# simonrw/rust-tensorflow-serving2

Measured on AMD Instinct MI355X. Metric: Predict RPCs/sec + p50 latency, ResNet-50 batch=1/32 at 1/2/4/8 MI355X, higher is better.
Workload: dtype bf16

## Files before the change

rust_tensorflow_serving2_amd/graph/fused.py:

```python
from __future__ import annotations

import os
from typing import Dict, List, Optional, Sequence, Set, Tuple

import numpy as np
import torch
import torch.nn.functional as F

from ..utils import tensors as T
from . import ops as O
from .ir import Graph, Node
from .placement import to_device, zeros

BF16 = torch.bfloat16


def _const(g: Graph, ref) -> Optional[torch.Tensor]:
    n = g.nodes.get(ref[0])
    if n is None or n.op != "Const" or n.value is None:
        return None
    v = n.value[ref[1]] if ref[1] < len(n.value) else None
    return v if isinstance(v, torch.Tensor) else None


# ... 686 lines not shown
        hc = (x.shape[1] + pt + pb - conv.kh) // conv.sh + 1
        wc = (x.shape[2] + pl + pr - conv.kw) // conv.sw + 1
        if pool.padding == "SAME":
            (ppt, ppb), (ppl, ppr) = O.tf_same_pads(hc, 3, 2), O.tf_same_pads(wc, 3, 2)
        else:
            ppt = ppb = ppl = ppr = 0
        kw = {}
        if pool.post is not None:
            sc, sh, act = pool.post
            kw = dict(post_scale=sc, post_shift=sh, post_act=ACT[act])
        x = x.contiguous() if x.dtype == torch.bfloat16 else x.float().contiguous()
        return [hip().stem_pool(x, conv.w, conv.b, pt, pb, pl, pr, ACT[conv.act],
                                ppt, ppb, ppl, ppr, **kw)]


O.OPS["_StemPool"] = _impl_op

CHAIN_SHAPES_ALL = {(64, 256, 64), (64, 256, 128), (128, 512, 128), (128, 512, 256)}
CHAIN_SHAPES_STAGE1 = {(64, 256, 64), (64, 256, 128)}
CHAIN_SHAPES_DEFAULT = CHAIN_SHAPES_ALL


class ChainConv:

    children = ("a", "b")

    def __init__(self, a: FusedConv, b: FusedConv):
        self.a, self.b = a, b
        self.use_hip = a.use_hip and b.use_hip
        self.name = a.name

    def __call__(self, ctx, node, ins):
        x = O.to_torch(ins[0])
        res = O.to_torch(ins[1]) if len(ins) > 1 else None
        a, b = self.a, self.b

        def split():
            y1 = a(ctx, node, ins)[0]
            return [y1, b(ctx, node, [y1])[0]]
        if not (self.use_hip and x.is_cuda and x.dim() == 4 and x.shape[-1] == a.cin):
            return split()
        from ..ops import ACT, hip, tuned_choice
        xb = _to_bf16(x).contiguous()
        rb = None if res is None else _to_bf16(res).contiguous()

        def chained():
            return list(hip().conv_chain(xb, a.w, a.b, rb, ACT[a.act], b.w, b.b, ACT[b.act]))
        key = ("chain", tuple(x.shape), a.cout, b.cout, res is not None, a.act, b.act)
        dflt = 1 if (a.cin, a.cout, b.cout) in CHAIN_SHAPES_STAGE1 else 0
        pick = tuned_choice(key, {1: chained, 0: split}, default=dflt)
        return chained() if pick == 1 else split()


O.OPS["_ChainConv"] = _impl_op
O.OPS["_FusedMatMulLN"] = _impl_op

_PASSTHROUGH = ("Identity", "Squeeze", "Reshape")


def fuse_classifier_head(g, order, fed, fetch_refs, device, opts):
    c = _Ctx(g, order, fed, fetch_refs, device, opts)

    def single(node) -> bool:
        return node.name not in c.fetch_nodes and len(c.cons.get(node.name, [])) == 1

    def walk(ref, chain):
        n = g.nodes.get(ref[0])
        while n is not None and n.op in _PASSTHROUGH and ref[1] == 0 and single(n) and n.inputs:
            chain.append(n)
            ref = n.inputs[0]
            n = g.nodes.get(ref[0])
        return ref, n

    for name in order:
        sm = g.nodes.get(name)
        if sm is None or sm.op != "_SoftmaxArgMax" or not sm.inputs:
            continue
        chain: List[Node] = []
        ref, mm = walk(sm.inputs[0], chain)
        if mm is None or mm.op != "_FusedMatMul" or ref[1] != 0 or len(mm.inputs) != 1 or not single(mm):
            continue
        impl = mm.attrs["_impl"]
        if impl.act != "none":
            continue
        chain.append(mm)
        ref, gap = walk(mm.inputs[0], chain)
        if gap is None or gap.op != "_GlobalAvgPool" or ref[1] != 0 or not single(gap):
            continue
        chain.append(gap)
        sm_impl = sm.attrs["_impl"]
        head = ClassifierHead(impl, sm_impl.cdt, c.use_hip)
        sm.op = "_ClassifierHead"
        sm.inputs = [gap.inputs[0]]
        sm.attrs = {"_impl": head}
        sm.ctrl = _merge_ctrl(chain + [sm])
        for n in chain:
            del g.nodes[n.name]
        c.refresh()


def fuse_stem_pool(g, order, fed, fetch_refs, device, opts):
    import os
    if os.environ.get("TFSERVE_STEM_POOL", "1") == "0":
        return
    c = _Ctx(g, order, fed, fetch_refs, device, opts)
    for name in order:
        p = g.nodes.get(name)
# ... 279 lines not shown
        impl = p.attrs["_impl"]
        if impl.post is not None or not impl.post_ok() or name in c.fetch_nodes:
            continue
        cons = c.cons.get(name, [])
        if any(i != 0 for _c, _p, i in cons):
            continue
        bns = [g.nodes[cn] for cn, _pos, _i in cons
               if g.nodes[cn].op.startswith("FusedBatchNorm") and g.nodes[cn].inputs[0] == (name, 0)]
        if len(bns) != 1:
            continue
        bn = bns[0]
        aff = _bn_affine(g, c, bn)
        if aff is None or aff[0].numel() != getattr(impl, "cout", aff[0].numel()):
            continue
        out_node, act = bn, "none"
        relu = c.only_consumer(bn.name)
        if relu is not None and relu.op == "Relu" and relu.name not in c.fetch_nodes:
            out_node, act = relu, "relu"
        elif bn.name in c.fetch_nodes:
            continue
        others = [cn for cn, _pos, _i in cons if cn != bn.name]
        if isinstance(impl, MaxPool) and others:
            continue
        mode = "dual" if others else "only"
        if isinstance(impl, MaxPool):
            impl.set_post(aff[0], aff[1], act, mode, device=c.device)
        else:
            impl.set_post(aff[0], aff[1], act, mode)
        new_ref = (name, 1 if mode == "dual" else 0)
        for cn, pos, _i in c.cons.get(out_node.name, []):
            g.nodes[cn].inputs[pos] = new_ref
        p.ctrl = _merge_ctrl([p, bn] + ([out_node] if out_node is not bn else []))
        del g.nodes[bn.name]
        if out_node is not bn:
            del g.nodes[out_node.name]
        c.refresh()


def _chainable_1x1(impl) -> bool:
    return (isinstance(impl, FusedConv) and impl.kh == 1 and impl.kw == 1 and impl.sh == 1 and impl.sw == 1 and
            not impl.c4 and impl.post is None and impl.act in ("relu", "none") and
            (impl.padding != "EXPLICIT" or not any(impl.pads)))


def fuse_conv_chain(g, order, fed, fetch_refs, device, opts):
    import os
    mode = os.environ.get("TFSERVE_CONV_CHAIN", "1")
    shapes = CHAIN_SHAPES_STAGE1 if os.environ.get("TFSERVE_CONV_CHAIN_SHAPES") == "stage1" else CHAIN_SHAPES_ALL
    c = _Ctx(g, order, fed, fetch_refs, device, opts)
    if mode == "0" or (not c.use_hip and mode != "force"):
        return
    for name in order:
        p = g.nodes.get(name)
        if p is None or p.op != "_FusedConv2D" or name in c.fetch_nodes:
            continue
        a = p.attrs["_impl"]
        if not _chainable_1x1(a):
            continue
        cons = c.cons.get(name, [])
        if any(i != 0 for _c, _p, i in cons):
            continue
        bs = [g.nodes[cn] for cn, pos, _i in cons
              if pos == 0 and g.nodes[cn].op == "_FusedConv2D" and len(g.nodes[cn].inputs) == 1 and
              cn not in c.fetch_nodes and _chainable_1x1(g.nodes[cn].attrs["_impl"])]
        if len(bs) != 1:
            continue
        bnode = bs[0]
        b = bnode.attrs["_impl"]
        if b.cin != a.cout or (a.cin, a.cout, b.cout) not in shapes:
            continue
        chain = ChainConv(a, b)
        p.op = "_ChainConv"
        p.attrs = {"_impl": chain}
        for cn, pos, _i in c.cons.get(bnode.name, []):
            g.nodes[cn].inputs[pos] = (name, 1)
        p.ctrl = _merge_ctrl([p, bnode])
        del g.nodes[bnode.name]
        c.refresh()


def default_passes(options=None):
    from .patterns import bert_passes, late_passes
    return [fuse_pools, fuse_softmax_argmax] + bert_passes() + [fuse_conv, fuse_dual_conv, fuse_post_activation,
                                                                 fuse_stem_pool, fuse_matmul,
                                                                 fuse_classifier_head, fuse_dense_softmax,
                                                                 fuse_conv_chain] + late_passes() + \
        [fuse_matmul_layernorm, defer_layernorm, release_weight_sources]
```

rust_tensorflow_serving2_amd/kernels/bindings.cpp:

```cpp
#include <cstdlib>
#include <algorithm>
#include <torch/extension.h>
#include <ATen/hip/impl/HIPGuardImplMasqueradingAsCUDA.h>
#include <ATen/hip/impl/HIPStreamMasqueradingAsCUDA.h>

#include "launch.h"
#include "cgemm.h"

namespace {

using torch::Tensor;

hipStream_t cur_stream(const Tensor& t) {
  return c10::hip::getCurrentHIPStreamMasqueradingAsCUDA(t.device().index()).stream();
}

void check(hipError_t e, const char* what) {
  TORCH_CHECK(e == hipSuccess, what, ": ", hipGetErrorString(e));
}

bool is_cgemm_cfg(int64_t cfg) {
  return cfg >= 0 && cfg < (1 << 20) && tfsk::cgemm_cfg_id(int(cfg));
}

// ... 375 lines not shown
    sh = post_shift->data_ptr<float>();
  }
  check(tfsk::maxpool_nhwc_launch(bf16p(x), bf16p_mut(y), N, H, W, C, KH, KW, SH, SW, PT, PL, Ho, Wo,
                                  cur_stream(x), sc, sh, int(post_act)), "maxpool");
  return y;
}

Tensor stem_pool(const Tensor& x, const Tensor& w, const Tensor& bias, int64_t PT, int64_t PB, int64_t PL, int64_t PR,
                 int64_t act, int64_t PPT, int64_t PPB, int64_t PPL, int64_t PPR,
                 const c10::optional<Tensor>& post_scale, const c10::optional<Tensor>& post_shift, int64_t post_act) {
  const bool xb16 = x.scalar_type() == at::kBFloat16;
  need(x, xb16 ? at::kBFloat16 : at::kFloat, "x");
  need(w, at::kBFloat16, "w");
  need(bias, at::kFloat, "bias");
  TORCH_CHECK(x.dim() == 4 && x.size(3) >= 1 && x.size(3) <= 4, "stem_pool: x must be NHWC with C <= 4");
  TORCH_CHECK(w.dim() == 2 && w.size(0) % 16 == 0 && w.size(0) >= 16 && w.size(0) <= 64 && w.size(1) >= 224 &&
              w.size(1) % 8 == 0, "stem_pool: w must be [cout in 16..64 step 16][>= 224, % 8]");
  TORCH_CHECK(bias.numel() == w.size(0), "stem_pool: bias must have cout entries");
  TORCH_CHECK(PT >= 0 && PB >= 0 && PL >= 0 && PR >= 0 && PPT >= 0 && PPT <= 2 && PPL >= 0 && PPL <= 2 &&
              PPB >= 0 && PPR >= 0, "stem_pool: bad padding");
  TORCH_CHECK(w.device() == x.device() && bias.device() == x.device(), "stem_pool: tensors on different devices");
  Tensor xin = x;
  if (xb16 && x.numel() % 2) {
    const int64_t avail = int64_t(x.storage().nbytes()) - int64_t(x.storage_offset()) * 2;
    if (avail < x.numel() * 2 + 2 || !x.is_contiguous()) {
      Tensor padded = torch::zeros({x.numel() + 1}, x.options());
      padded.narrow(0, 0, x.numel()).copy_(x.reshape({-1}));
      xin = padded.narrow(0, 0, x.numel()).view(x.sizes());
    }
  }
  c10::hip::HIPGuardMasqueradingAsCUDA guard(x.device());
  const int N = x.size(0), H = x.size(1), W = x.size(2), C = x.size(3), cout = w.size(0);
  const int Hc = (H + PT + PB - 7) / 2 + 1, Wc = (W + PL + PR - 7) / 2 + 1;
  TORCH_CHECK(Hc >= 1 && Wc >= 1, "stem_pool: input smaller than the filter");
  const int Hp = (Hc + PPT + PPB - 3) / 2 + 1, Wp = (Wc + PPL + PPR - 3) / 2 + 1;
  TORCH_CHECK(Hp >= 1 && Wp >= 1, "stem_pool: conv output smaller than the pool window");
  Tensor y = torch::empty({N, Hp, Wp, cout}, x.options().dtype(at::kBFloat16));
  const float* sc = nullptr;
  const float* sh = nullptr;
  if (post_scale.has_value()) {
    TORCH_CHECK(post_shift.has_value(), "post_scale needs post_shift");
    need(*post_scale, at::kFloat, "post_scale");
    need(*post_shift, at::kFloat, "post_shift");
    TORCH_CHECK(post_scale->numel() == cout && post_shift->numel() == cout, "post scale / shift must have cout entries");
    sc = post_scale->data_ptr<float>();
    sh = post_shift->data_ptr<float>();
  }
  check(tfsk::stem_pool_launch(xin.data_ptr(), xb16, bf16p(w), int(w.size(1)), bias.data_ptr<float>(), bf16p_mut(y), N,
                               H, W, C, cout, int(PT), int(PL), Hc, Wc, int(PPT), int(PPL), Hp, Wp, int(act), sc, sh,
                               int(post_act), cur_stream(x)), "stem_pool");
  return y;
}

std::vector<Tensor> conv_chain(const Tensor& x, const Tensor& w1, const Tensor& b1,
                               const c10::optional<Tensor>& residual, int64_t act1, const Tensor& w2,
                               const Tensor& b2, int64_t act2) {
  need(x, at::kBFloat16, "x");
  need(w1, at::kBFloat16, "w1");
  need(w2, at::kBFloat16, "w2");
  need(b1, at::kFloat, "b1");
  need(b2, at::kFloat, "b2");
  TORCH_CHECK(x.dim() == 4, "conv_chain: x must be NHWC");
  const int K1 = x.size(3), N1 = w1.size(0), N2 = w2.size(0);
  TORCH_CHECK(w1.dim() == 2 && w2.dim() == 2 && w1.size(1) >= K1 && w2.size(1) >= N1 && w1.size(1) % 8 == 0 &&
                  w2.size(1) % 8 == 0, "conv_chain: w1 [N1][>= K1], w2 [N2][>= N1]");
  TORCH_CHECK(tfsk::conv_chain_supported(K1, N1, N2), "conv_chain: unsupported shape K1=", K1, " N1=", N1, " N2=", N2);
  TORCH_CHECK(b1.numel() == N1 && b2.numel() == N2, "conv_chain: bias sizes");
  TORCH_CHECK(w1.device() == x.device() && w2.device() == x.device() && b1.device() == x.device() &&
                  b2.device() == x.device(), "conv_chain: tensors on different devices");
  const uint16_t* rp = nullptr;
  if (residual.has_value()) {
    need(*residual, at::kBFloat16, "residual");
    TORCH_CHECK(residual->dim() == 4 && residual->size(0) == x.size(0) && residual->size(1) == x.size(1) &&
                    residual->size(2) == x.size(2) && residual->size(3) == N1, "conv_chain: residual [n][h][w][N1]");
    rp = bf16p(*residual);
  }
  c10::hip::HIPGuardMasqueradingAsCUDA guard(x.device());
  const int M = x.size(0) * x.size(1) * x.size(2);
  Tensor y1 = torch::empty({x.size(0), x.size(1), x.size(2), N1}, x.options());
  Tensor y2 = torch::empty({x.size(0), x.size(1), x.size(2), N2}, x.options());
  check(tfsk::conv_chain_launch(bf16p(x), bf16p(w1), int(w1.size(1)), b1.data_ptr<float>(), rp, bf16p_mut(y1),
                                bf16p(w2), int(w2.size(1)), b2.data_ptr<float>(), bf16p_mut(y2), M, K1, N1, N2,
                                int(act1), int(act2), cur_stream(x)),
        "conv_chain");
  return {y1, y2};
}

Tensor global_avgpool(const Tensor& x, const c10::optional<Tensor>& out) {
  need(x, at::kBFloat16, "x");
  TORCH_CHECK(x.dim() == 4 && x.size(3) % 8 == 0, "global_avgpool: NHWC with C % 8 == 0");
  c10::hip::HIPGuardMasqueradingAsCUDA guard(x.device());
  const int N = x.size(0), HW = x.size(1) * x.size(2), C = x.size(3);
  Tensor y = out.has_value() ? *out : torch::empty({N, C}, x.options());
  need(y, at::kBFloat16, "out");
  check(tfsk::global_avgpool_nhwc_launch(bf16p(x), bf16p_mut(y), N, HW, C, cur_stream(x)), "gap");
  return y;
}

std::vector<Tensor> softmax_argmax(const Tensor& logits, bool want_probs, bool want_classes,
                                   const c10::optional<Tensor>& probs_out,
                                   const c10::optional<Tensor>& classes_out) {
  TORCH_CHECK(logits.is_cuda() && logits.dim() >= 1 && logits.stride(-1) == 1 &&
                  (logits.is_contiguous() || logits.dim() == 2),
              "logits must be a GPU tensor with unit column stride (contiguous, or 2-D with a row stride)");
  const bool bf = logits.scalar_type() == at::kBFloat16;
  TORCH_CHECK(bf || logits.scalar_type() == at::kFloat, "logits must be f32 or bf16");
  c10::hip::HIPGuardMasqueradingAsCUDA guard(logits.device());
  const int cols = logits.size(-1);
  const int rows = logits.numel() / cols;
  const long ld = logits.dim() == 2 ? long(logits.stride(0)) : long(cols);
  TORCH_CHECK(ld >= cols, "logits row stride");
  Tensor probs, classes;
  if (want_probs) {
    probs = probs_out.has_value() ? *probs_out : torch::empty(logits.sizes(), logits.options().dtype(at::kFloat));
    need(probs, at::kFloat, "probs");
  }
  if (want_classes) {
    auto sz = logits.sizes().vec();
    sz.pop_back();
    classes = classes_out.has_value() ? *classes_out : torch::empty(sz, logits.options().dtype(at::kLong));
    need(classes, at::kLong, "classes");
  }
  check(tfsk::softmax_argmax_launch(logits.data_ptr(), bf, want_probs ? probs.data_ptr<float>() : nullptr,
                                    want_classes ? classes.data_ptr<int64_t>() : nullptr, rows, cols, ld,
                                    cur_stream(logits)), "softmax_argmax");
  return {probs, classes};
}

std::tuple<Tensor, Tensor, bool> classifier_head_impl(const Tensor& x, const Tensor& w, const Tensor& bias, int64_t n,
                                                      int64_t probs_host, int64_t classes_host);

std::vector<Tensor> classifier_head(const Tensor& x, const Tensor& w, const Tensor& bias, int64_t n) {
  auto r = classifier_head_impl(x, w, bias, n, 0, 0);
  return {std::get<0>(r), std::get<1>(r)};
}

std::tuple<Tensor, Tensor, bool> classifier_head_impl(const Tensor& x, const Tensor& w, const Tensor& bias, int64_t n,
// ... 182 lines not shown
  }
  if (pos.has_value()) {
    need(*pos, at::kBFloat16, "pos");
    TORCH_CHECK(pos->dim() == 2 && pos->size(1) == Hd && pos->size(0) >= seq, "embed_ln: pos shape");
    pp = bf16p(*pos);
  }
  auto shape = ids.sizes().vec();
  shape.push_back(Hd);
  Tensor y = torch::empty(shape, word.options());
  check(tfsk::embed_ln_launch(ids.data_ptr<int>(), tt, bf16p(word), pp, tp, gamma.data_ptr<float>(),
                              beta.data_ptr<float>(), bf16p_mut(y), tokens, seq, Hd, word.size(0), ntypes,
                              float(eps), cur_stream(ids)), "embed_ln");
  return y;
}

Tensor attention(const Tensor& qkv, const c10::optional<Tensor>& mask_bias, int64_t heads, double scale,
                 const c10::optional<Tensor>& out, int64_t mask_bstride, int64_t mask_qstride) {
  need(qkv, at::kBFloat16, "qkv");
  TORCH_CHECK(qkv.dim() == 3, "qkv must be [B, S, 3*H*D]");
  c10::hip::HIPGuardMasqueradingAsCUDA guard(qkv.device());
  const int B = qkv.size(0), S = qkv.size(1), HD3 = qkv.size(2);
  TORCH_CHECK(HD3 % (3 * heads) == 0, "qkv width must be 3*heads*head_dim");
  const int D = HD3 / (3 * heads);
  TORCH_CHECK(D == 64, "attention kernel supports head_dim 64");
  TORCH_CHECK(S >= 1 && S <= tfsk::kMaxAttentionSeq, "attention kernel supports 1 <= S <= ", tfsk::kMaxAttentionSeq);
  const float* mb = nullptr;
  if (mask_bias.has_value()) {
    need(*mask_bias, at::kFloat, "mask_bias");
    const int64_t last = int64_t(B - 1) * mask_bstride + int64_t(S - 1) * mask_qstride + (S - 1);
    TORCH_CHECK(mask_bstride >= 0 && mask_qstride >= 0 && last < mask_bias->numel(),
                "mask strides exceed the mask tensor");
    mb = mask_bias->data_ptr<float>();
  }
  Tensor y = out.has_value() ? *out : torch::empty({B, S, heads * D}, qkv.options());
  need(y, at::kBFloat16, "out");
  check(tfsk::attention_launch(bf16p(qkv), mb, bf16p_mut(y), B, S, heads, D, float(scale), mask_bstride,
                               mask_qstride, cur_stream(qkv)),
        "attention");
  return y;
}

}

PYBIND11_MODULE(TORCH_EXTENSION_NAME, m) {
  m.doc() = "gfx950 HIP kernels (MFMA implicit-GEMM conv/GEMM, attention, norms, pooling)";
  m.def("conv2d", &conv2d, "NHWC implicit-GEMM conv (+bias +residual +act)", py::arg("x"), py::arg("w"),
        py::arg("bias"), py::arg("residual"), py::arg("kh"), py::arg("kw"), py::arg("sh"), py::arg("sw"),
        py::arg("pt"), py::arg("pb"), py::arg("pl"), py::arg("pr"), py::arg("act") = 0, py::arg("cfg") = 0,
        py::arg("out") = py::none(), py::arg("out_f32") = false, py::arg("splits") = 1,
        py::arg("post_scale") = py::none(), py::arg("post_shift") = py::none(), py::arg("post_act") = 0,
        py::arg("out2") = py::none(), py::arg("post_only") = false);
  m.def("conv_chain", &conv_chain, "expand 1x1 (+residual, act) -> next reduce 1x1 (+act) in one kernel",
        py::arg("x"), py::arg("w1"), py::arg("b1"), py::arg("residual"), py::arg("act1"), py::arg("w2"),
        py::arg("b2"), py::arg("act2"));
  m.def("conv_chain_supported", [](int64_t k1, int64_t n1, int64_t n2) {
    return tfsk::conv_chain_supported(int(k1), int(n1), int(n2));
  });
  m.def("conv2d_dual", &conv2d_dual, "act(conv1x1(h) + conv1x1_stride(x) + bias) as one K-concatenated GEMM",
        py::arg("h"), py::arg("x"), py::arg("w"), py::arg("bias"), py::arg("sh"), py::arg("sw"), py::arg("act") = 0,
        py::arg("cfg") = 36, py::arg("out") = py::none(), py::arg("splits") = 1,
        py::arg("post_scale") = py::none(), py::arg("post_shift") = py::none(), py::arg("post_act") = 0,
        py::arg("out2") = py::none(), py::arg("post_only") = false);
  m.def("linear_lnx", &linear_lnx,
        "GEMM whose A / residual rows are LayerNorm inputs (statistics as partials), optionally "
        "returning its own rows' partials: {y, partials}",
        py::arg("x"), py::arg("w"), py::arg("bias"), py::arg("residual"), py::arg("act"), py::arg("cfg"),
        py::arg("out_f32") = false, py::arg("out") = py::none(), py::arg("a_st") = py::none(),
        py::arg("a_colsum") = py::none(), py::arg("a_eps") = 1e-12, py::arg("r_st") = py::none(),
        py::arg("r_gamma") = py::none(), py::arg("r_beta") = py::none(), py::arg("r_eps") = 1e-12,
        py::arg("stats") = false);
  m.def("linear", &linear,"x @ w^T (+bias +residual +act)", py::arg("x"), py::arg("w"), py::arg("bias"),
        py::arg("residual") = py::none(), py::arg("act") = 0, py::arg("cfg") = 0, py::arg("out_f32") = false,
        py::arg("alpha") = 1.0, py::arg("out") = py::none(), py::arg("splits") = 1);
  m.def("stem_pool", &stem_pool, py::arg("x"), py::arg("w"), py::arg("bias"), py::arg("pt"), py::arg("pb"),
        py::arg("pl"), py::arg("pr"), py::arg("act"), py::arg("ppt"), py::arg("ppb"), py::arg("ppl"), py::arg("ppr"),
        py::arg("post_scale") = py::none(), py::arg("post_shift") = py::none(), py::arg("post_act") = 0);
  m.def("maxpool", &maxpool, py::arg("x"), py::arg("kh"), py::arg("kw"), py::arg("sh"), py::arg("sw"),
        py::arg("pt"), py::arg("pb"), py::arg("pl"), py::arg("pr"), py::arg("out") = py::none(),
        py::arg("post_scale") = py::none(), py::arg("post_shift") = py::none(), py::arg("post_act") = 0);
  m.def("global_avgpool", &global_avgpool, py::arg("x"), py::arg("out") = py::none());
  m.def("classifier_head", &classifier_head, "softmax/argmax(mean_hw(x) @ w^T + bias)[:, :n]", py::arg("x"),
        py::arg("w"), py::arg("bias"), py::arg("n"));
  m.def("softmax_argmax", &softmax_argmax, py::arg("logits"), py::arg("want_probs") = true,
        py::arg("want_classes") = true, py::arg("probs_out") = py::none(), py::arg("classes_out") = py::none());
  m.def("dense_softmax", &dense_softmax, "softmax(x @ w[:n]^T + bias[:n]) for n <= 16 labels (x f32)",
        py::arg("x"), py::arg("w"), py::arg("bias"), py::arg("n"));
  m.def("key_mask_adder", &key_mask_adder, "(one - m) * scale as f32", py::arg("m"), py::arg("one"),
        py::arg("scale"));
  m.def("cast_bf16", &cast_bf16, py::arg("x"), py::arg("out") = py::none());
  m.def("ingest_c4", &ingest_c4, "fp32 NHWC (C<=4) -> bf16 NHWC C=4", py::arg("x"), py::arg("out") = py::none());
  m.def("ingest_c4_padded", &ingest_c4_padded, "fp32 NHWC (C<=4) -> zero-bordered bf16 RGBA [N][Hp][Wp][4]",
        py::arg("x"), py::arg("hp"), py::arg("wp"), py::arg("pt"), py::arg("pl"));
  m.def("ingest_c4_from_host", &ingest_c4_from_host, "ingest_c4 reading a pinned host tensor (zero-copy)",
        py::arg("x"), py::arg("out"));
  m.def("h2d_rows", &h2d_rows, py::arg("host"), py::arg("dev"),
        "copy a pinned host tensor into a device tensor with a kernel (system-scope loads; capturable)");
  m.def("cast_bf16_from_host", &cast_bf16_from_host, "fp32 pinned host tensor -> bf16 device tensor",
        py::arg("x"), py::arg("out"));
  m.def("linear_ln", &linear_ln, "LN(x @ w^T + bias + residual) * gamma + beta, whole rows per workgroup",
        py::arg("x"), py::arg("w"), py::arg("bias"), py::arg("residual"), py::arg("gamma"), py::arg("beta"),
        py::arg("eps"), py::arg("bm") = 32, py::arg("out") = py::none());
  m.def("linear_ln_supported", [](int64_t M, int64_t N, int64_t K, int64_t bm) {
    return tfsk::lngemm_supported(int(M), int(N), int(K), int(bm));
  });
  m.def("layernorm", &layernorm, py::arg("x"), py::arg("residual"), py::arg("gamma"), py::arg("beta"),
        py::arg("eps"), py::arg("out") = py::none());
  m.def("embed_ln", &embed_ln, py::arg("ids"), py::arg("type_ids"), py::arg("word"), py::arg("pos"),
// ... 70 lines not shown
```

rust_tensorflow_serving2_amd/kernels/chain.hip:

```cpp
#include "gemm_common.h"

namespace tfsk {
namespace {

using namespace gemm;

struct ChainArgs {
  const uint16_t* x;
  const uint16_t* w1;
  const float* b1;
  const uint16_t* res;
  uint16_t* y1;
  const uint16_t* w2;
  const float* b2;
  uint16_t* y2;
  int M, ldw1, ldw2;
  float lo1, lo2;
};

constexpr int kBM = 64, kNT = 256, kStgLd = 68;

template <int K1, int N1, int N2>
struct CH {
  static constexpr int KT1 = K1 / KT, KT2 = N1 / KT;
  static constexpr int A_BYTES = KT1 * kBM * KT * 2;
  static constexpr int W1_BYTES = KT1 * N1 * KT * 2;
  static constexpr int P1 = A_BYTES + W1_BYTES;
  static constexpr int CHAIN = KT2 * kBM * KT * 2;
  static constexpr int STG = 4 * 16 * kStgLd * 4;
  static constexpr int S2 = N2 <= 128 ? 3 : 2;
  static constexpr int W2_SLOT = N2 * KT * 2;
  static constexpr int RING_OFF = CHAIN;
  static constexpr int P23 = CHAIN + (STG > S2 * W2_SLOT ? STG : S2 * W2_SLOT);
  static constexpr int LDS = P1 > P23 ? P1 : P23;
  static constexpr int WN1 = N1 / 4, TN1 = WN1 / 16, U1 = WN1 / 64;
  static constexpr int WN2 = N2 / 2, TN2 = WN2 / 16;
  static constexpr int UW2 = WN2 < 64 ? WN2 : 64, U2 = WN2 / UW2;
  static constexpr int APW = KT1 * (kBM / 8) / 4, W1PW = KT1 * (N1 / 8) / 4, W2PW = N2 / 32;
  static_assert(K1 % KT == 0 && N1 % 256 == 0 && N2 % 64 == 0, "chain shape");
  static_assert(LDS <= 160 * 1024, "LDS budget");
  static_assert((S2 - 2) * W2PW < 64, "vmcnt range");
};

template <int K1, int N1, int N2>
__global__ __launch_bounds__(256, 1) void conv_chain_kernel(ChainArgs p) {
  using G = CH<K1, N1, N2>;
  extern __shared__ __attribute__((aligned(16))) char smem[];
  typedef __attribute__((address_space(3))) void* lds_ptr_t;
  const int tid = threadIdx.x, lane = tid & 63;
  const int wid = __builtin_amdgcn_readfirstlane(tid >> 6);
  const int fr = lane & 15, fq = lane >> 4;
  const int prow = lane >> 3;
  const uint32_t kc = uint32_t(((lane & 7) ^ prow) * 8);
  const int m0 = xcd_remap(blockIdx.x, gridDim.x) * kBM;
  const int M = p.M;

  const __amdgpu_buffer_rsrc_t rsX = __builtin_amdgcn_make_buffer_rsrc(
      const_cast<uint16_t*>(p.x), 0, int(long(M) * K1 * 2), 0x00020000);
  const __amdgpu_buffer_rsrc_t rsW1 = __builtin_amdgcn_make_buffer_rsrc(
      const_cast<uint16_t*>(p.w1), 0, int(long(N1) * p.ldw1 * 2), 0x00020000);
  const __amdgpu_buffer_rsrc_t rsW2 = __builtin_amdgcn_make_buffer_rsrc(
      const_cast<uint16_t*>(p.w2), 0, int(long(N2) * p.ldw2 * 2), 0x00020000);

#pragma unroll
  for (int j = 0; j < G::APW; ++j) {
    const int q = wid * G::APW + j;
    const int kt = q / (kBM / 8), pc = q % (kBM / 8);
    const int m = m0 + pc * 8 + prow;
    const uint32_t v = m < M ? (uint32_t(m) * K1 + uint32_t(kt * KT) + kc) * 2u : kOOB;
    __builtin_amdgcn_raw_ptr_buffer_load_lds(rsX, (lds_ptr_t)(smem + kt * kBM * KT * 2 + pc * 1024), 16, v, 0, 0, 0);
  }
#pragma unroll
  for (int j = 0; j < G::W1PW; ++j) {
    const int q = wid * G::W1PW + j;
    const int kt = q / (N1 / 8), pc = q % (N1 / 8);
    const int n = pc * 8 + prow;
    const uint32_t v = (uint32_t(n) * uint32_t(p.ldw1) + uint32_t(kt * KT) + kc) * 2u;
    __builtin_amdgcn_raw_ptr_buffer_load_lds(rsW1, (lds_ptr_t)(smem + G::A_BYTES + kt * N1 * KT * 2 + pc * 1024), 16,
                                             v, 0, 0, 0);
  }

  const int c8 = lane & 7, rl = lane >> 3;
  float4 bias1[G::U1][2];
#pragma unroll
  for (int c = 0; c < G::U1; ++c) {
    const int n = wid * G::WN1 + c * 64 + c8 * 8;
    bias1[c][0] = *reinterpret_cast<const float4*>(p.b1 + n);
    bias1[c][1] = *reinterpret_cast<const float4*>(p.b1 + n + 4);
  }
  const __amdgpu_buffer_rsrc_t rsR = __builtin_amdgcn_make_buffer_rsrc(
      const_cast<uint16_t*>(p.res), 0, p.res ? int(long(M) * N1 * 2) : 0, 0x00020000);
  u32x4 rr[4][G::U1][2];
#pragma unroll
  for (int i = 0; i < 4; ++i)
#pragma unroll
    for (int c = 0; c < G::U1; ++c)
#pragma unroll
      for (int k = 0; k < 2; ++k) {
        const int m = m0 + i * 16 + rl + 8 * k;
        const int n = wid * G::WN1 + c * 64 + c8 * 8;
        const uint32_t v = m < M ? (uint32_t(m) * N1 + uint32_t(n)) * 2u : kOOB;
        rr[i][c][k] = __builtin_amdgcn_raw_buffer_load_b128(rsR, v, 0, 0);
      }

  wait_vmcnt<0>();
  __syncthreads();

  f32x4 acc[4][G::TN1];
#pragma unroll
  for (int i = 0; i < 4; ++i)
#pragma unroll
    for (int j = 0; j < G::TN1; ++j) acc[i][j] = f32x4{0.f, 0.f, 0.f, 0.f};
  const uint32_t ro0 = uint32_t((fr * KT + ((fq ^ (fr & 7)) * 8)) * 2);
  const uint32_t ro1 = uint32_t((fr * KT + (((4 + fq) ^ (fr & 7)) * 8)) * 2);
#pragma unroll
  for (int kt = 0; kt < G::KT1; ++kt) {
    const char* sa = smem + kt * kBM * KT * 2;
    const char* sb = smem + G::A_BYTES + kt * N1 * KT * 2 + wid * G::WN1 * KT * 2;
#pragma unroll
    for (int kk = 0; kk < 2; ++kk) {
      bf16x8 af[4], bfr[G::TN1];
#pragma unroll
      for (int i = 0; i < 4; ++i) af[i] = *reinterpret_cast<const bf16x8*>(sa + (kk ? ro1 : ro0) + i * 16 * KT * 2);
// ... 105 lines not shown
        for (int kk = 0; kk < 2; ++kk) {
          bf16x8 af[2], bfr[G::TN2];
#pragma unroll
          for (int i = 0; i < 2; ++i) af[i] = *reinterpret_cast<const bf16x8*>(sa + (kk ? ra1 : ra0) + i * 16 * KT * 2);
#pragma unroll
          for (int j = 0; j < G::TN2; ++j)
            bfr[j] = *reinterpret_cast<const bf16x8*>(sb + (kk ? rb1 : rb0) + j * 16 * KT * 2);
#pragma unroll
          for (int i = 0; i < 2; ++i)
#pragma unroll
            for (int j = 0; j < G::TN2; ++j)
              acc2[i][j] = __builtin_amdgcn_mfma_f32_16x16x32_bf16(af[i], bfr[j], acc2[i][j], 0, 0, 0);
        }
      }
    }
  }

  __syncthreads();
  const __amdgpu_buffer_rsrc_t rsY2 =
      __builtin_amdgcn_make_buffer_rsrc(p.y2, 0, int(long(M) * N2 * 2), 0x00020000);
#pragma unroll
  for (int i = 0; i < 2; ++i) {
#pragma unroll
    for (int c = 0; c < G::U2; ++c) {
#pragma unroll
      for (int jj = 0; jj < G::UW2 / 16; ++jj)
#pragma unroll
        for (int r = 0; r < 4; ++r)
          stg[(fq * 4 + r) * kStgLd + jj * 16 + fr] = acc2[i][c * (G::UW2 / 16) + jj][r];
      __builtin_amdgcn_wave_barrier();
#pragma unroll
      for (int k = 0; k < IT2; ++k) {
        const int item = lane + 64 * k;
        const int rloc = item / CPR2, cc = item % CPR2;
        const float* src = stg + rloc * kStgLd + cc * 8;
        const float4 lo = *reinterpret_cast<const float4*>(src);
        const float4 hi = *reinterpret_cast<const float4*>(src + 4);
        const int n = wn2 * G::WN2 + c * G::UW2 + cc * 8;
        const u32x4 b0 = b2v[c][k][0], b1 = b2v[c][k][1];
        auto f = [](uint32_t u) { return __uint_as_float(u); };
        u32x4 ov;
        ov.x = pack_bf16x2(fmaxf(lo.x + f(b0.x), p.lo2), fmaxf(lo.y + f(b0.y), p.lo2));
        ov.y = pack_bf16x2(fmaxf(lo.z + f(b0.z), p.lo2), fmaxf(lo.w + f(b0.w), p.lo2));
        ov.z = pack_bf16x2(fmaxf(hi.x + f(b1.x), p.lo2), fmaxf(hi.y + f(b1.y), p.lo2));
        ov.w = pack_bf16x2(fmaxf(hi.z + f(b1.z), p.lo2), fmaxf(hi.w + f(b1.w), p.lo2));
        const int m = m0 + wm2 * 32 + i * 16 + rloc;
        __builtin_amdgcn_raw_buffer_store_b128(ov, rsY2, m < M ? (uint32_t(m) * N2 + uint32_t(n)) * 2u : kOOB, 0, 0);
      }
      __builtin_amdgcn_wave_barrier();
    }
  }
}

template <int K1, int N1, int N2>
hipError_t launch_chain(const ChainArgs& a, hipStream_t s) {
  using G = CH<K1, N1, N2>;
  hipError_t e = ensure_dyn_lds(reinterpret_cast<const void*>(&conv_chain_kernel<K1, N1, N2>), G::LDS);
  if (e != hipSuccess) return e;
  const int tiles = (a.M + kBM - 1) / kBM;
  hipLaunchKernelGGL((conv_chain_kernel<K1, N1, N2>), dim3(tiles), dim3(kNT), G::LDS, s, a);
  return hipGetLastError();
}

}

bool conv_chain_supported(int K1, int N1, int N2) {
  return (K1 == 64 && N1 == 256 && (N2 == 64 || N2 == 128)) || (K1 == 128 && N1 == 512 && (N2 == 128 || N2 == 256));
}

hipError_t conv_chain_launch(const uint16_t* x, const uint16_t* w1, int ldw1, const float* b1, const uint16_t* res,
                             uint16_t* y1, const uint16_t* w2, int ldw2, const float* b2, uint16_t* y2, int M, int K1,
                             int N1, int N2, int act1, int act2, hipStream_t s) {
  if (M <= 0) return hipSuccess;
  if (!conv_chain_supported(K1, N1, N2) || ldw1 < K1 || ldw1 % 8 || ldw2 < N1 || ldw2 % 8) return hipErrorInvalidValue;
  if ((act1 != kActNone && act1 != kActRelu) || (act2 != kActNone && act2 != kActRelu)) return hipErrorInvalidValue;
  if (long(M) * N1 * 2 >= 0x7fffffffL) return hipErrorInvalidValue;
  ChainArgs a{x, w1, b1, res, y1, w2, b2, y2, M, ldw1, ldw2, act1 == kActRelu ? 0.f : -INFINITY,
              act2 == kActRelu ? 0.f : -INFINITY};
  if (K1 == 64 && N1 == 256 && N2 == 64) return launch_chain<64, 256, 64>(a, s);
  if (K1 == 64 && N1 == 256 && N2 == 128) return launch_chain<64, 256, 128>(a, s);
  if (K1 == 128 && N1 == 512 && N2 == 128) return launch_chain<128, 512, 128>(a, s);
  return launch_chain<128, 512, 256>(a, s);
}

}
```

rust_tensorflow_serving2_amd/kernels/launch.h:

```cpp
#pragma once
#include <hip/hip_runtime.h>
#include <stdint.h>

namespace tfsk {

struct IGemmArgs {
  const void* a;
  const uint16_t* b;
  int M, N, K;
  int lda, ldb;
  int H, W, C, KH, KW, SH, SW, PT, PL, Ho, Wo;
  const float* bias;
  const uint16_t* residual;
  int ldr;
  int act;
  void* out;
  int ldc;
  int out_f32;
  float alpha;
  int splits;
  int kt_per_split;
  float* ws;
  int64_t a_bytes;
  int64_t b_bytes;
// ... 4 lines not shown
  void* out2;
  const float* scale2;
  const float* shift2;
  int act2;
  int* counters;
  long long* trace;
  int trace_cap;
  int epi_f32;
  float* st_out;
  const float* a_st;
  const float* a_colsum;
  int a_parts;
  float a_eps;
  const float* r_st;
  const float* r_gamma;
  const float* r_beta;
  int r_parts;
  float r_eps;
};

int* splitk_counters(int n, hipStream_t s);
void splitk_counters_prepare(hipStream_t s);
void splitk_counters_set_owner(int64_t owner);
void splitk_counters_add_stream(int64_t owner, hipStream_t s);
int64_t splitk_counters_release(int64_t owner);
int64_t splitk_counters_reclaim();
int64_t splitk_counters_pending();
int64_t splitk_counters_captured_in_use();

enum AMode : int { kADense = 0, kAIm2col = 1, kAStemF32 = 2, kAStem7x7x3 = 3, kAC4 = 4, kADual = 5 };

hipError_t ingest_c4_launch(const float* x, uint16_t* y, int64_t pixels, int C, hipStream_t stream);

hipError_t ingest_c4_pad_launch(const float* x, uint16_t* y, int N, int H, int W, int C, int Hp, int Wp, int pt,
                               int pl, hipStream_t stream);

hipError_t splitk_reduce_launch(const IGemmArgs& args, hipStream_t stream);

constexpr int kNumIGemmConfigs = 17;
int igemm_config_bm(int cfg);
int igemm_config_bn(int cfg);
int igemm_config_stages(int cfg);
int igemm_config_bk(int cfg);
hipError_t igemm_launch(const IGemmArgs& args, int a_mode, int cfg, hipStream_t stream);

hipError_t stem_pool_launch(const void* x, bool x_bf16, const uint16_t* w, int ldw, const float* bias, uint16_t* y,
                            int N, int H, int W, int C, int cout, int pt, int pl, int Hc, int Wc, int ppt, int ppl,
                            int Hp, int Wp, int act, const float* pscale, const float* pshift, int pact,
                            hipStream_t s);
bool conv_chain_supported(int K1, int N1, int N2);
hipError_t conv_chain_launch(const uint16_t* x, const uint16_t* w1, int ldw1, const float* b1, const uint16_t* res,
                             uint16_t* y1, const uint16_t* w2, int ldw2, const float* b2, uint16_t* y2, int M, int K1,
                             int N1, int N2, int act1, int act2, hipStream_t s);
hipError_t maxpool_nhwc_launch(const uint16_t* x, uint16_t* y, int N, int H, int W, int C,
                               int KH, int KW, int SH, int SW, int PT, int PL, int Ho, int Wo,
                               hipStream_t stream, const float* scale = nullptr, const float* shift = nullptr,
                               int act = 0);
hipError_t global_avgpool_nhwc_launch(const uint16_t* x, uint16_t* y, int N, int HW, int C,
                                      hipStream_t stream);
hipError_t classifier_head_launch(const uint16_t* x, const uint16_t* w, const float* bias, float* ws,
                                  float* probs, int64_t* classes, int M, int HW, int K, int Np, int N,
                                  hipStream_t s, int* counter = nullptr, float* probs_h = nullptr,
                                  int64_t* classes_h = nullptr);
size_t classifier_head_ws_floats(int M, int K, int Np);
bool classifier_head_one_launch(int M, int HW, int K, int Np, int N);
hipError_t dense_softmax_launch(const float* x, int ldx, const uint16_t* w, int ldw, const float* bias,
                                float* probs, int rows, int N, int K, hipStream_t s);
hipError_t key_mask_adder_launch(const void* m, int is_int, float one, float scale, float* out, int64_t n,
                                 hipStream_t s);
hipError_t softmax_argmax_launch(const void* logits, int in_bf16, float* probs, int64_t* classes,
                                 int rows, int cols, long ld, hipStream_t stream);
hipError_t cast_f32_bf16_launch(const float* x, uint16_t* y, int64_t n, hipStream_t stream);
hipError_t cast_bf16_f32_launch(const uint16_t* x, float* y, int64_t n, hipStream_t stream);
int epi_f32_env();
hipError_t h2d_rows_launch(const void* host, void* dev, int64_t bytes, hipStream_t stream);

hipError_t layernorm_launch(const uint16_t* x, const uint16_t* r, const float* gamma, const float* beta,
                            uint16_t* y, int rows, int cols, float eps, hipStream_t stream);
hipError_t embed_ln_launch(const int* ids, const int* type_ids, const uint16_t* word,
                           const uint16_t* pos, const uint16_t* type, const float* gamma,
                           const float* beta, uint16_t* y, int tokens, int seq, int hidden,
                           int vocab, int ntypes, float eps, hipStream_t stream);
struct LnGemmArgs {
  const uint16_t* x = nullptr;
  const uint16_t* w = nullptr;
  const float* bias = nullptr;
  const uint16_t* r = nullptr;
  const float* gamma = nullptr;
  const float* beta = nullptr;
  uint16_t* y = nullptr;
  int M = 0, N = 0, K = 0, ldx = 0;
  float eps = 1e-12f;
};
bool lngemm_supported(int M, int N, int K, int bm);
hipError_t lngemm_launch(const LnGemmArgs& a, int bm, hipStream_t stream);
constexpr int kMaxAttentionSeq = 4096;
hipError_t attention_launch(const uint16_t* qkv, const float* mask_bias, uint16_t* ctx, int B, int S,
                            int H, int D, float scale, long mask_bstride, long mask_qstride,
                            hipStream_t stream);
void attention_set_trace(long long* trace, int cap);
int attention_set_plds(int mode);

}
```

Before: 56170.

## Fuse dual-source projection conv with following reduce 1x1 into one chain kernel

Adds a dual-source variant of the conv-chain kernel. It reads one k-tile from each of two 64-channel tensors, so the first ResNet block's expand conv, with its projection shortcut folded in, runs together with the next block's reduce 1x1 in one launch. A new graph pass case rewrites matching _FusedDualConv -> _FusedConv2D pairs into _ChainDualConv, picked by the tuner with default on. This removes a kernel launch and a global round trip of the intermediate for that shape. The cost is extra kernel code, and the fused kernel may schedule worse than two separate launches. It also adds optional preallocated output tensors to the chain bindings.

```diff
diff --git a/rust_tensorflow_serving2_amd/graph/fused.py b/rust_tensorflow_serving2_amd/graph/fused.py
--- a/rust_tensorflow_serving2_amd/graph/fused.py
+++ b/rust_tensorflow_serving2_amd/graph/fused.py
@@ -762,7 +762,37 @@
         return chained() if pick == 1 else split()
 
 
+class ChainDualConv:
+
+    children = ("a", "b")
+
+    def __init__(self, a: FusedDualConv, b: FusedConv, node_a: Node, node_b: Node):
+        self.a, self.b = a, b
+        self.use_hip = a.use_hip and b.use_hip
+        self.name = a.name
+        self.subs = [(a, node_a), (b, node_b)]
+
+    def __call__(self, ctx, node, ins):
+        h, x = O.to_torch(ins[0]), O.to_torch(ins[1])
+        a, b = self.a, self.b
+
+        def split():
+            y1 = a(ctx, node, ins)[0]
+            return [y1, b(ctx, node, [y1])[0]]
+        if not (self.use_hip and h.is_cuda and h.dim() == 4 and h.shape == x.shape and h.shape[-1] == a.c1):
+            return split()
+        from ..ops import ACT, hip, tuned_choice
+        hb, xb = _to_bf16(h).contiguous(), _to_bf16(x).contiguous()
+
+        def chained():
+            return list(hip().conv_chain_dual(hb, xb, a.w, a.b, ACT[a.act], b.w, b.b, ACT[b.act]))
+        key = ("chain_dual", tuple(h.shape), a.cout, b.cout, a.act, b.act)
+        pick = tuned_choice(key, {1: chained, 0: split}, default=1)
+        return chained() if pick == 1 else split()
+
+
 O.OPS["_ChainConv"] = _impl_op
+O.OPS["_ChainDualConv"] = _impl_op
 O.OPS["_FusedMatMulLN"] = _impl_op
 
 _PASSTHROUGH = ("Identity", "Squeeze", "Reshape")
@@ -1148,10 +1178,15 @@
         return
     for name in order:
         p = g.nodes.get(name)
-        if p is None or p.op != "_FusedConv2D" or name in c.fetch_nodes:
+        if p is None or p.op not in ("_FusedConv2D", "_FusedDualConv") or name in c.fetch_nodes:
             continue
         a = p.attrs["_impl"]
-        if not _chainable_1x1(a):
+        dual = p.op == "_FusedDualConv"
+        if dual:
+            if not (a.use_hip and a.sh == a.sw == 1 and a.c1 == a.c2 == 64 and a.cout == 256 and a.post is None and
+                    a.act in ("relu", "none")):
+                continue
+        elif not _chainable_1x1(a):
             continue
         cons = c.cons.get(name, [])
         if any(i != 0 for _c, _p, i in cons):
@@ -1163,10 +1198,17 @@
             continue
         bnode = bs[0]
         b = bnode.attrs["_impl"]
-        if b.cin != a.cout or (a.cin, a.cout, b.cout) not in shapes:
-            continue
-        chain = ChainConv(a, b)
-        p.op = "_ChainConv"
+        if dual:
+            if b.cin != a.cout or b.cout != 64 or not b.use_hip:
+                continue
+            import copy
+            chain = ChainDualConv(a, b, copy.copy(p), bnode)
+            p.op = "_ChainDualConv"
+        else:
+            if b.cin != a.cout or (a.cin, a.cout, b.cout) not in shapes:
+                continue
+            chain = ChainConv(a, b)
+            p.op = "_ChainConv"
         p.attrs = {"_impl": chain}
         for cn, pos, _i in c.cons.get(bnode.name, []):
             g.nodes[cn].inputs[pos] = (name, 1)
diff --git a/rust_tensorflow_serving2_amd/kernels/bindings.cpp b/rust_tensorflow_serving2_amd/kernels/bindings.cpp
--- a/rust_tensorflow_serving2_amd/kernels/bindings.cpp
+++ b/rust_tensorflow_serving2_amd/kernels/bindings.cpp
@@ -451,9 +451,18 @@
   return y;
 }
 
+Tensor chain_out(const c10::optional<Tensor>& out, const Tensor& x, int64_t M, int64_t N, const char* name) {
+  if (!out.has_value()) return torch::empty({x.size(0), x.size(1), x.size(2), N}, x.options());
+  need(*out, at::kBFloat16, name);
+  TORCH_CHECK(out->is_contiguous() && out->dim() >= 2 && out->size(-1) == N && out->numel() >= M * N &&
+                  out->device() == x.device(), "conv_chain: ", name, " must be contiguous [>= M rows][N]");
+  return *out;
+}
+
 std::vector<Tensor> conv_chain(const Tensor& x, const Tensor& w1, const Tensor& b1,
                                const c10::optional<Tensor>& residual, int64_t act1, const Tensor& w2,
-                               const Tensor& b2, int64_t act2) {
+                               const Tensor& b2, int64_t act2, const c10::optional<Tensor>& y1o,
+                               const c10::optional<Tensor>& y2o) {
   need(x, at::kBFloat16, "x");
   need(w1, at::kBFloat16, "w1");
   need(w2, at::kBFloat16, "w2");
@@ -476,12 +485,41 @@
   }
   c10::hip::HIPGuardMasqueradingAsCUDA guard(x.device());
   const int M = x.size(0) * x.size(1) * x.size(2);
-  Tensor y1 = torch::empty({x.size(0), x.size(1), x.size(2), N1}, x.options());
-  Tensor y2 = torch::empty({x.size(0), x.size(1), x.size(2), N2}, x.options());
+  Tensor y1 = chain_out(y1o, x, M, N1, "y1");
+  Tensor y2 = chain_out(y2o, x, M, N2, "y2");
   check(tfsk::conv_chain_launch(bf16p(x), bf16p(w1), int(w1.size(1)), b1.data_ptr<float>(), rp, bf16p_mut(y1),
                                 bf16p(w2), int(w2.size(1)), b2.data_ptr<float>(), bf16p_mut(y2), M, K1, N1, N2,
                                 int(act1), int(act2), cur_stream(x)),
         "conv_chain");
+  return {y1, y2};
+}
+
+std::vector<Tensor> conv_chain_dual(const Tensor& h, const Tensor& x, const Tensor& w1, const Tensor& b1, int64_t act1,
+                                    const Tensor& w2, const Tensor& b2, int64_t act2,
+                                    const c10::optional<Tensor>& y1o, const c10::optional<Tensor>& y2o) {
+  need(h, at::kBFloat16, "h");
+  need(x, at::kBFloat16, "x");
+  need(w1, at::kBFloat16, "w1");
+  need(w2, at::kBFloat16, "w2");
+  need(b1, at::kFloat, "b1");
+  need(b2, at::kFloat, "b2");
+  TORCH_CHECK(h.dim() == 4 && x.dim() == 4 && h.sizes() == x.sizes() && h.size(3) == 64,
+              "conv_chain_dual: h and x must both be [n][h][w][64]");
+  TORCH_CHECK(w1.dim() == 2 && w2.dim() == 2, "conv_chain_dual: w1 [N1][>= 128], w2 [N2][>= N1]");
+  const int N1 = w1.size(0), N2 = w2.size(0);
+  TORCH_CHECK(N1 == 256 && N2 == 64 && w1.size(1) >= 128 && w2.size(1) >= N1 && w1.size(1) % 8 == 0 &&
+                  w2.size(1) % 8 == 0, "conv_chain_dual: w1 [256][>= 128], w2 [64][>= 256]");
+  TORCH_CHECK(b1.numel() == N1 && b2.numel() == N2, "conv_chain_dual: bias sizes");
+  TORCH_CHECK(x.device() == h.device() && w1.device() == h.device() && w2.device() == h.device() &&
+                  b1.device() == h.device() && b2.device() == h.device(), "conv_chain_dual: tensors on different devices");
+  c10::hip::HIPGuardMasqueradingAsCUDA guard(h.device());
+  const int M = h.size(0) * h.size(1) * h.size(2);
+  Tensor y1 = chain_out(y1o, h, M, N1, "y1");
+  Tensor y2 = chain_out(y2o, h, M, N2, "y2");
+  check(tfsk::conv_chain_dual_launch(bf16p(h), bf16p(x), bf16p(w1), int(w1.size(1)), b1.data_ptr<float>(),
+                                     bf16p_mut(y1), bf16p(w2), int(w2.size(1)), b2.data_ptr<float>(), bf16p_mut(y2), M,
+                                     N1, N2, int(act1), int(act2), cur_stream(h)),
+        "conv_chain_dual");
   return {y1, y2};
 }
 
@@ -770,7 +808,11 @@
         py::arg("out2") = py::none(), py::arg("post_only") = false);
   m.def("conv_chain", &conv_chain, "expand 1x1 (+residual, act) -> next reduce 1x1 (+act) in one kernel",
         py::arg("x"), py::arg("w1"), py::arg("b1"), py::arg("residual"), py::arg("act1"), py::arg("w2"),
-        py::arg("b2"), py::arg("act2"));
+        py::arg("b2"), py::arg("act2"), py::arg("y1") = py::none(), py::arg("y2") = py::none());
+  m.def("conv_chain_dual", &conv_chain_dual,
+        "expand 1x1 over [h | x] (projection shortcut folded in, act) -> next reduce 1x1 (+act) in one kernel",
+        py::arg("h"), py::arg("x"), py::arg("w1"), py::arg("b1"), py::arg("act1"), py::arg("w2"), py::arg("b2"),
+        py::arg("act2"), py::arg("y1") = py::none(), py::arg("y2") = py::none());
   m.def("conv_chain_supported", [](int64_t k1, int64_t n1, int64_t n2) {
     return tfsk::conv_chain_supported(int(k1), int(n1), int(n2));
   });
diff --git a/rust_tensorflow_serving2_amd/kernels/chain.hip b/rust_tensorflow_serving2_amd/kernels/chain.hip
--- a/rust_tensorflow_serving2_amd/kernels/chain.hip
+++ b/rust_tensorflow_serving2_amd/kernels/chain.hip
@@ -7,6 +7,7 @@
 
 struct ChainArgs {
   const uint16_t* x;
+  const uint16_t* x2;
   const uint16_t* w1;
   const float* b1;
   const uint16_t* res;
@@ -42,8 +43,9 @@
   static_assert((S2 - 2) * W2PW < 64, "vmcnt range");
 };
 
-template <int K1, int N1, int N2>
+template <int K1, int N1, int N2, bool DUAL = false>
 __global__ __launch_bounds__(256, 1) void conv_chain_kernel(ChainArgs p) {
+  static_assert(!DUAL || K1 == 2 * KT, "dual source: one k-tile from each tensor");
   using G = CH<K1, N1, N2>;
   extern __shared__ __attribute__((aligned(16))) char smem[];
   typedef __attribute__((address_space(3))) void* lds_ptr_t;
@@ -55,8 +57,11 @@
   const int m0 = xcd_remap(blockIdx.x, gridDim.x) * kBM;
   const int M = p.M;
 
+  constexpr int LDX = DUAL ? KT : K1;
   const __amdgpu_buffer_rsrc_t rsX = __builtin_amdgcn_make_buffer_rsrc(
-      const_cast<uint16_t*>(p.x), 0, int(long(M) * K1 * 2), 0x00020000);
+      const_cast<uint16_t*>(p.x), 0, int(long(M) * LDX * 2), 0x00020000);
+  const __amdgpu_buffer_rsrc_t rsX2 = __builtin_amdgcn_make_buffer_rsrc(
+      const_cast<uint16_t*>(DUAL ? p.x2 : p.x), 0, int(long(M) * LDX * 2), 0x00020000);
   const __amdgpu_buffer_rsrc_t rsW1 = __builtin_amdgcn_make_buffer_rsrc(
       const_cast<uint16_t*>(p.w1), 0, int(long(N1) * p.ldw1 * 2), 0x00020000);
   const __amdgpu_buffer_rsrc_t rsW2 = __builtin_amdgcn_make_buffer_rsrc(
@@ -67,8 +72,9 @@
     const int q = wid * G::APW + j;
     const int kt = q / (kBM / 8), pc = q % (kBM / 8);
     const int m = m0 + pc * 8 + prow;
-    const uint32_t v = m < M ? (uint32_t(m) * K1 + uint32_t(kt * KT) + kc) * 2u : kOOB;
-    __builtin_amdgcn_raw_ptr_buffer_load_lds(rsX, (lds_ptr_t)(smem + kt * kBM * KT * 2 + pc * 1024), 16, v, 0, 0, 0);
+    const uint32_t v = m < M ? (uint32_t(m) * LDX + uint32_t(DUAL ? 0 : kt * KT) + kc) * 2u : kOOB;
+    __builtin_amdgcn_raw_ptr_buffer_load_lds(DUAL && kt ? rsX2 : rsX, (lds_ptr_t)(smem + kt * kBM * KT * 2 + pc * 1024),
+                                             16, v, 0, 0, 0);
   }
 #pragma unroll
   for (int j = 0; j < G::W1PW; ++j) {
@@ -280,13 +286,13 @@
   }
 }
 
-template <int K1, int N1, int N2>
+template <int K1, int N1, int N2, bool DUAL = false>
 hipError_t launch_chain(const ChainArgs& a, hipStream_t s) {
   using G = CH<K1, N1, N2>;
-  hipError_t e = ensure_dyn_lds(reinterpret_cast<const void*>(&conv_chain_kernel<K1, N1, N2>), G::LDS);
+  hipError_t e = ensure_dyn_lds(reinterpret_cast<const void*>(&conv_chain_kernel<K1, N1, N2, DUAL>), G::LDS);
   if (e != hipSuccess) return e;
   const int tiles = (a.M + kBM - 1) / kBM;
-  hipLaunchKernelGGL((conv_chain_kernel<K1, N1, N2>), dim3(tiles), dim3(kNT), G::LDS, s, a);
+  hipLaunchKernelGGL((conv_chain_kernel<K1, N1, N2, DUAL>), dim3(tiles), dim3(kNT), G::LDS, s, a);
   return hipGetLastError();
 }
 
@@ -303,7 +309,7 @@
   if (!conv_chain_supported(K1, N1, N2) || ldw1 < K1 || ldw1 % 8 || ldw2 < N1 || ldw2 % 8) return hipErrorInvalidValue;
   if ((act1 != kActNone && act1 != kActRelu) || (act2 != kActNone && act2 != kActRelu)) return hipErrorInvalidValue;
   if (long(M) * N1 * 2 >= 0x7fffffffL) return hipErrorInvalidValue;
-  ChainArgs a{x, w1, b1, res, y1, w2, b2, y2, M, ldw1, ldw2, act1 == kActRelu ? 0.f : -INFINITY,
+  ChainArgs a{x, nullptr, w1, b1, res, y1, w2, b2, y2, M, ldw1, ldw2, act1 == kActRelu ? 0.f : -INFINITY,
               act2 == kActRelu ? 0.f : -INFINITY};
   if (K1 == 64 && N1 == 256 && N2 == 64) return launch_chain<64, 256, 64>(a, s);
   if (K1 == 64 && N1 == 256 && N2 == 128) return launch_chain<64, 256, 128>(a, s);
@@ -311,4 +317,16 @@
   return launch_chain<128, 512, 256>(a, s);
 }
 
-}
+hipError_t conv_chain_dual_launch(const uint16_t* h, const uint16_t* x, const uint16_t* w1, int ldw1, const float* b1,
+                                  uint16_t* y1, const uint16_t* w2, int ldw2, const float* b2, uint16_t* y2, int M,
+                                  int N1, int N2, int act1, int act2, hipStream_t s) {
+  if (M <= 0) return hipSuccess;
+  if (N1 != 256 || N2 != 64 || ldw1 < 2 * KT || ldw1 % 8 || ldw2 < N1 || ldw2 % 8) return hipErrorInvalidValue;
+  if ((act1 != kActNone && act1 != kActRelu) || (act2 != kActNone && act2 != kActRelu)) return hipErrorInvalidValue;
+  if (long(M) * N1 * 2 >= 0x7fffffffL) return hipErrorInvalidValue;
+  ChainArgs a{h, x, w1, b1, nullptr, y1, w2, b2, y2, M, ldw1, ldw2, act1 == kActRelu ? 0.f : -INFINITY,
+              act2 == kActRelu ? 0.f : -INFINITY};
+  return launch_chain<128, 256, 64, true>(a, s);
+}
+
+}
diff --git a/rust_tensorflow_serving2_amd/kernels/launch.h b/rust_tensorflow_serving2_amd/kernels/launch.h
--- a/rust_tensorflow_serving2_amd/kernels/launch.h
+++ b/rust_tensorflow_serving2_amd/kernels/launch.h
@@ -80,6 +80,9 @@
 hipError_t conv_chain_launch(const uint16_t* x, const uint16_t* w1, int ldw1, const float* b1, const uint16_t* res,
                              uint16_t* y1, const uint16_t* w2, int ldw2, const float* b2, uint16_t* y2, int M, int K1,
                              int N1, int N2, int act1, int act2, hipStream_t s);
+hipError_t conv_chain_dual_launch(const uint16_t* h, const uint16_t* x, const uint16_t* w1, int ldw1, const float* b1,
+                                  uint16_t* y1, const uint16_t* w2, int ldw2, const float* b2, uint16_t* y2, int M,
+                                  int N1, int N2, int act1, int act2, hipStream_t s);
 hipError_t maxpool_nhwc_launch(const uint16_t* x, uint16_t* y, int N, int H, int W, int C,
                                int KH, int KW, int SH, int SW, int PT, int PL, int Ho, int Wo,
                                hipStream_t stream, const float* scale = nullptr, const float* shift = nullptr,
```

Measured after the change: 55950. Within noise of the previous version (-0.4%).
